# lim0606/pytorch-ardae-vae

Measured on AMD Instinct MI355X. Metric: AR-DAE-VAE train-steps/sec (batch 512, nz_cdae 256) on dbMNIST, higher is better.
Workload: dtype f32; 1 GPU; BASELINE config #2: MNISTIPVAE mlp z=32 h=256 + cDAE mlp-grad h=256 L=3, global batch 512, nz_cdae 256 (131072 rows), dynamic binarisation on device, 1 cDAE + 1 VAE update per step; global_batch=512, nz_cdae=256, per_gpu_batch=512, parallelism=dp1

## Files before the change

pytorch-ardae-vae_amd/csrc/wgrad_x9.hip:

```cpp
#include <stdlib.h>

#include <type_traits>

#include "profile.h"
#include "wgrad.h"
#include "wgrad_wide_tiles.h"

namespace ardae {
namespace {

typedef __bf16 bf16x8 __attribute__((ext_vector_type(8)));
typedef float f32x8 __attribute__((ext_vector_type(8)));

constexpr int XT = 256;
constexpr int XRC = 16;
constexpr int X_PLANE_BYTES = 2 * XT * 16;
constexpr int X_OP_BYTES = 3 * X_PLANE_BYTES;
constexpr int X_BUF_BYTES = 2 * X_OP_BYTES;

__device__ __forceinline__ void xload1(float& dst, unsigned voff, const float* sbase) {
  asm volatile("s_nop 4\n\tglobal_load_dword %0, %1, %2" : "+v"(dst) : "v"(voff), "s"(sbase) : "memory");
}
__device__ __forceinline__ void xload4(f32x4& dst, unsigned voff, const float* sbase) {
  asm volatile("s_nop 4\n\tglobal_load_dwordx4 %0, %1, %2" : "+v"(dst) : "v"(voff), "s"(sbase) : "memory");
}
template <int N>
__device__ __forceinline__ void xwait() { asm volatile("s_waitcnt vmcnt(%0)" : : "n"(N) : "memory"); }
__device__ __forceinline__ void take_landed(const float& loaded, unsigned& top, float& copy) {
  asm volatile("v_and_b32 %0, 0xffff0000, %2\n\tv_mov_b32 %1, %2" : "=&v"(top), "=&v"(copy) : "v"(loaded));
}
__device__ __forceinline__ void take_landed(const f32x4& loaded, f32x4& copy) {
  asm volatile("v_mov_b32 %0, %4\n\tv_mov_b32 %1, %5\n\tv_mov_b32 %2, %6\n\tv_mov_b32 %3, %7"
               : "=&v"(copy[0]), "=&v"(copy[1]), "=&v"(copy[2]), "=&v"(copy[3])
               : "v"(loaded[0]), "v"(loaded[1]), "v"(loaded[2]), "v"(loaded[3]));
}

struct Cut3 { unsigned h, m, l; };
__device__ __forceinline__ Cut3 cut3(float x) {
  Cut3 c;
  c.h = __float_as_uint(x) & 0xffff0000u;
  const float r1 = x - __uint_as_float(c.h);
  c.m = __float_as_uint(r1) & 0xffff0000u;
  c.l = __float_as_uint(r1 - __uint_as_float(c.m));
  return c;
}
__device__ __forceinline__ unsigned pack_hi(unsigned even, unsigned odd) { return __builtin_amdgcn_perm(odd, even, 0x07060302u); }
typedef unsigned u32x4 __attribute__((ext_vector_type(4)));

template <int N, class F>
__device__ __forceinline__ void static_for(F&& f) {
  if constexpr (N > 0) {
    static_for<N - 1>(f);
    f(std::integral_constant<int, N - 1>{});
  }
}
constexpr int X9_PA[9] = {2, 1, 2, 0, 2, 1, 0, 1, 0}, X9_PB[9] = {2, 2, 1, 2, 0, 1, 1, 0, 0};

struct X9Chunk {
  const float* g; const float* x; const float* rs;
  int ldg, ldx;
  float fb, fr;
};

__global__ __launch_bounds__(256, 1) void wgrad_x9_kernel(const WwBatchDev batch) {
  extern __shared__ __attribute__((aligned(16))) unsigned char lds[];
  const int tid = threadIdx.x, lane = tid & 63;
  const int wave = __builtin_amdgcn_readfirstlane(tid >> 6);
  const int l31 = lane & 31, hh = lane >> 5;
  const int wo = wave >> 1, wi = wave & 1;
  const int ti = (int)blockIdx.x / batch.splits, split = (int)blockIdx.x - ti * batch.splits;
  const WwTile T = batch.t[ti];

  const int cpp = T.M / XRC;
  const int ctot = cpp * T.npairs;
  const int cps = (ctot + batch.splits - 1) / batch.splits;
  const int c_begin = split * cps;
  const int c_end = c_begin + cps < ctot ? c_begin + cps : ctot;

  auto chunk_at = [&](int ch) {
    X9Chunk c;
    const int cc = ch < c_end ? ch : c_end - 1;
    const int pr = cc >= cpp ? 1 : 0;
    const int m0 = (cc - pr * cpp) * XRC;
    c.ldg = pr ? T.ldG[1] : T.ldG[0];
    c.ldx = pr ? T.ldX[1] : T.ldX[0];
    c.g = (pr ? T.G[1] : T.G[0]) + (size_t)m0 * c.ldg + T.o0;
    c.x = (pr ? T.X[1] : T.X[0]) + (size_t)m0 * c.ldx + T.i0;
    const bool vec = T.want_vec && pr == T.bias_pair && ch < c_end;
    c.fb = vec ? 1.f : 0.f;
    c.fr = (vec && T.rowscale) ? 1.f : 0.f;
    c.rs = T.rowscale ? T.rowscale + m0 : c.g;
    return c;
  };
  auto issue_loads = [&](const X9Chunk& c, float (&g)[XRC], float (&x)[XRC], f32x4 (&rs)[4]) {
    const float* pg = c.g;
    const float* px = c.x;
#pragma unroll
    for (int j = 0; j < XRC; ++j) {
      xload1(g[j], (unsigned)tid * 4u, pg); pg += c.ldg;
      if ((j & 3) == 3) xload4(rs[j >> 2], 0u, c.rs + (j & ~3));
    }
#pragma unroll
    for (int j = 0; j < XRC; ++j) { xload1(x[j], (unsigned)tid * 4u, px); px += c.ldx; }
  };
  float bsum = 0.f, rsum = 0.f;
  auto write_group = [&](const u32x4& h, const u32x4& m, const u32x4& l, int op, int kg, unsigned char* buf) {
    unsigned char* p = buf + op * X_OP_BYTES + (kg * XT + tid) * 16;
    *reinterpret_cast<u32x4*>(p) = h;
    *reinterpret_cast<u32x4*>(p + X_PLANE_BYTES) = m;
    *reinterpret_cast<u32x4*>(p + 2 * X_PLANE_BYTES) = l;
  };
  auto stage_group = [&](const float (&v)[XRC], int op, int kg, unsigned char* buf) {
    u32x4 h, m, l;
#pragma unroll
    for (int q = 0; q < 4; ++q) {
      const Cut3 e = cut3(v[8 * kg + 2 * q]), o = cut3(v[8 * kg + 2 * q + 1]);
      h[q] = pack_hi(e.h, o.h); m[q] = pack_hi(e.m, o.m); l[q] = pack_hi(e.l, o.l);
    }
    write_group(h, m, l, op, kg, buf);
  };

  f32x16 acc[4][4];
#pragma unroll
  for (int a = 0; a < 4; ++a)
#pragma unroll
    for (int b = 0; b < 4; ++b)
#pragma unroll
      for (int r = 0; r < 16; ++r) acc[a][b][r] = 0.f;

  if (c_begin < c_end) {
    float gc[XRC], xc[XRC];
    f32x4 rsc[4];
#pragma unroll
    for (int j = 0; j < XRC; ++j) gc[j] = xc[j] = 0.f;
#pragma unroll
    for (int q = 0; q < 4; ++q) rsc[q] = f32x4{0.f, 0.f, 0.f, 0.f};
    {
      const X9Chunk c0 = chunk_at(c_begin);
      issue_loads(c0, gc, xc, rsc);
      asm volatile("s_waitcnt vmcnt(0)" ::: "memory");
#pragma unroll
      for (int j = 0; j < XRC; ++j) asm volatile("" : "+v"(gc[j]), "+v"(xc[j]));
#pragma unroll
      for (int q = 0; q < 4; ++q) asm volatile("" : "+v"(rsc[q]));
      {
        float s0 = 0.f, r0 = 0.f;
#pragma unroll
        for (int j = 0; j < XRC; ++j) { s0 += gc[j]; r0 += gc[j] * rsc[j >> 2][j & 3]; }
        bsum += s0 * c0.fb; rsum += r0 * c0.fr;
      }
      stage_group(gc, 0, 0, lds); stage_group(gc, 0, 1, lds); stage_group(xc, 1, 0, lds); stage_group(xc, 1, 1, lds);
      issue_loads(chunk_at(c_begin + 1), gc, xc, rsc);
      __syncthreads();
    }
    int buf = 0;
    bf16x8 Af[3][4], Bf[3][4];
    auto read_plane = [&](auto pp, const unsigned char* from) {
      constexpr int p = decltype(pp)::value;
      static_for<4>([&](auto aa) {
        constexpr int a = decltype(aa)::value;
        Af[p][a] = *reinterpret_cast<const bf16x8*>(from + p * X_PLANE_BYTES + (hh * XT + wo * 128 + a * 32 + l31) * 16);
      });
      static_for<4>([&](auto bb) {
        constexpr int b = decltype(bb)::value;
        Bf[p][b] = *reinterpret_cast<const bf16x8*>(from + X_OP_BYTES + p * X_PLANE_BYTES + (hh * XT + wi * 128 + b * 32 + l31) * 16);
      });
    };
    using I0 = std::integral_constant<int, 0>;
    using I1 = std::integral_constant<int, 1>;
    using I2 = std::integral_constant<int, 2>;
    read_plane(I2{}, lds);
    read_plane(I1{}, lds);
    X9Chunk c1 = chunk_at(c_begin + 1);
#pragma unroll 1
    for (int ch = c_begin; ch < c_end; ++ch) {
      unsigned char* cur = lds + buf * X_BUF_BYTES;
      unsigned char* oth = lds + (buf ^ 1) * X_BUF_BYTES;
      const X9Chunk c2 = chunk_at(ch + 2);
      const float* pgn = c2.g;
      const float* pxn = c2.x;
      u32x4 sh, sm, sl;
      Cut3 ce{0u, 0u, 0u}, co{0u, 0u, 0u};
      float r1 = 0.f, vv = 0.f, cs = 0.f, cr = 0.f;
      f32x4 rsv = {0.f, 0.f, 0.f, 0.f};
      static_for<144>([&](auto nn) {
        constexpr int n = decltype(nn)::value, s = n >> 4, idx = n & 15, a = idx >> 2, b = idx & 3;
        acc[a][b] = __builtin_amdgcn_mfma_f32_32x32x16_bf16(Af[X9_PA[s]][a], Bf[X9_PB[s]][b], acc[a][b], 0, 0, 0);
        __builtin_amdgcn_sched_barrier(0);
        if constexpr (n == 0) {
          read_plane(I0{}, cur);
          __builtin_amdgcn_sched_barrier(0);
        }
        if constexpr (n < 124) {
          constexpr int grp = n / 31, r = n % 31;
          if constexpr (r < 28) {
            constexpr int pr = r / 7, slot = r % 7, e = 8 * grp + 2 * pr + (slot >= 3 ? 1 : 0), op = e >> 4, j = e & 15;
            float& v = op ? xc[j] : gc[j];
            if constexpr (slot == 0 || slot == 3) {
              xwait<35>();
              Cut3& c = slot == 0 ? ce : co;
              take_landed(v, c.h, vv);
              r1 = vv - __uint_as_float(c.h);
              if constexpr (op == 0) cs += vv;
            } else if constexpr (slot == 1 || slot == 4) {
              Cut3& c = slot == 1 ? ce : co;
              c.m = __float_as_uint(r1) & 0xffff0000u;
              c.l = __float_as_uint(r1 - __uint_as_float(c.m));
              if constexpr (op == 0) {
                if constexpr ((j & 3) == 0) { xwait<31>(); take_landed(rsc[j >> 2], rsv); }
                cr += vv * rsv[j & 3];
              }
            } else if constexpr (slot == 2 || slot == 5) {
              if constexpr (op == 0) {
                xload1(v, (unsigned)tid * 4u, pgn); pgn += c2.ldg;
                if constexpr ((j & 3) == 3) xload4(rsc[j >> 2], 0u, c2.rs + (j & ~3));
              } else {
                xload1(v, (unsigned)tid * 4u, pxn); pxn += c2.ldx;
              }
            } else {
              sh[pr] = pack_hi(ce.h, co.h); sm[pr] = pack_hi(ce.m, co.m); sl[pr] = pack_hi(ce.l, co.l);
            }
          } else {
            constexpr int pl = r - 28;
            unsigned char* p = oth + (grp >> 1) * X_OP_BYTES + ((grp & 1) * XT + tid) * 16 + pl * X_PLANE_BYTES;
            *reinterpret_cast<u32x4*>(p) = pl == 0 ? sh : pl == 1 ? sm : sl;
          }
          __builtin_amdgcn_sched_barrier(0);
        }
        if constexpr (n == 124) {
          __syncthreads();
          __builtin_amdgcn_sched_barrier(0);
        }
        if constexpr (n == 125) {
          read_plane(I2{}, oth);
          __builtin_amdgcn_sched_barrier(0);
        }
        if constexpr (n == 128) {
          read_plane(I1{}, oth);
          __builtin_amdgcn_sched_barrier(0);
        }
      });
      bsum += cs * c1.fb; rsum += cr * c1.fr;
      buf ^= 1;
      c1 = c2;
    }
    asm volatile("s_waitcnt vmcnt(0)" ::: "memory");
  }

  float* __restrict__ part = T.partial + (size_t)split * T.O * T.I;
#pragma unroll
  for (int a = 0; a < 4; ++a) {
#pragma unroll
    for (int b = 0; b < 4; ++b) {
      const int i = T.i0 + wi * 128 + b * 32 + l31;
#pragma unroll
      for (int r = 0; r < 16; ++r) {
        const int o = T.o0 + wo * 128 + a * 32 + (r & 3) + 8 * (r >> 2) + 4 * hh;
        part[(size_t)o * T.I + i] = acc[a][b][r];
      }
    }
  }
  if (T.want_vec && T.i0 == 0) {
    T.partial_vec[((size_t)split * 2 + 0) * T.O + T.o0 + tid] = bsum;
    T.partial_vec[((size_t)split * 2 + 1) * T.O + T.o0 + tid] = rsum;
  }
}

}

bool wgrad_x9_eligible(const WgradProblem& p) {
  static const bool off = debug_knob("ARDAE_WGRAD_X9") && atoi(debug_knob("ARDAE_WGRAD_X9")) == 0;
  if (off || p.O % XT || p.I % XT || p.M % XRC || p.M < 64 * 32) return false;
  for (int k = 0; k < p.npairs; ++k)
    if ((int64_t)p.ldG[k] * XRC * 4 >= (int64_t)1 << 31 || (int64_t)p.ldX[k] * XRC * 4 >= (int64_t)1 << 31) return false;
  return true;
}

int launch_wgrad_x9(const WwBatchDev& b, hipStream_t st) {
  static const bool attr_set = [] {
    return hipFuncSetAttribute(reinterpret_cast<const void*>(wgrad_x9_kernel), hipFuncAttributeMaxDynamicSharedMemorySize, 2 * X_BUF_BYTES) == hipSuccess;
  }();
  ARDAE_CHECK_ARG(attr_set, "wgrad_x9: cannot reserve %d bytes of LDS", 2 * X_BUF_BYTES);
  hipLaunchKernelGGL(wgrad_x9_kernel, dim3(b.ntiles * b.splits), dim3(256), 2 * X_BUF_BYTES, st, b);
  return 0;
}

}
```

Measured before the change: 223.7 train-steps/sec.

## Add 8-wave variant of x9 weight-gradient kernel and make it default

Adds a 512-thread version of the 3-way bf16-split weight-gradient MFMA kernel. Each wave now owns a 128x64 output sub-tile instead of 128x128, and half the waves stage G while the other half stage X, so per-thread global loads and split/pack work are halved. Row scales are read through scalar constant-address loads. The goal is more latency hiding and higher MFMA issue rate per CU. The cost is extra LDS A-fragment reads per MFMA and a barrier shared by more waves. The old 4-wave kernel can still be selected with a debug knob.

```diff
diff --git a/pytorch-ardae-vae_amd/csrc/wgrad_x9.hip b/pytorch-ardae-vae_amd/csrc/wgrad_x9.hip
--- a/pytorch-ardae-vae_amd/csrc/wgrad_x9.hip
+++ b/pytorch-ardae-vae_amd/csrc/wgrad_x9.hip
@@ -1,3 +1,4 @@
+#include <stdint.h>
 #include <stdlib.h>
 
 #include <type_traits>
@@ -46,6 +47,7 @@
 }
 __device__ __forceinline__ unsigned pack_hi(unsigned even, unsigned odd) { return __builtin_amdgcn_perm(odd, even, 0x07060302u); }
 typedef unsigned u32x4 __attribute__((ext_vector_type(4)));
+typedef __attribute__((address_space(4))) const float ConstF;
 
 template <int N, class F>
 __device__ __forceinline__ void static_for(F&& f) {
@@ -61,6 +63,39 @@
   int ldg, ldx;
   float fb, fr;
 };
+
+__device__ __forceinline__ X9Chunk x9_chunk_at(const WwTile& T, int ch, int c_end, int cpp) {
+  X9Chunk c;
+  const int cc = ch < c_end ? ch : c_end - 1;
+  const int pr = cc >= cpp ? 1 : 0;
+  const int m0 = (cc - pr * cpp) * XRC;
+  c.ldg = pr ? T.ldG[1] : T.ldG[0];
+  c.ldx = pr ? T.ldX[1] : T.ldX[0];
+  c.g = (pr ? T.G[1] : T.G[0]) + (size_t)m0 * c.ldg + T.o0;
+  c.x = (pr ? T.X[1] : T.X[0]) + (size_t)m0 * c.ldx + T.i0;
+  const bool vec = T.want_vec && pr == T.bias_pair && ch < c_end;
+  c.fb = vec ? 1.f : 0.f;
+  c.fr = (vec && T.rowscale) ? 1.f : 0.f;
+  c.rs = T.rowscale ? T.rowscale + m0 : c.g;
+  return c;
+}
+
+template <int NB>
+__device__ __forceinline__ void x9_store_partial(const WwTile& T, int split, const f32x16 (&acc)[4][NB], int o_w, int i_w, int l31, int hh) {
+  float* __restrict__ part = T.partial + (size_t)split * T.O * T.I;
+#pragma unroll
+  for (int a = 0; a < 4; ++a) {
+#pragma unroll
+    for (int b = 0; b < NB; ++b) {
+      const int i = T.i0 + i_w + b * 32 + l31;
+#pragma unroll
+      for (int r = 0; r < 16; ++r) {
+        const int o = T.o0 + o_w + a * 32 + (r & 3) + 8 * (r >> 2) + 4 * hh;
+        part[(size_t)o * T.I + i] = acc[a][b][r];
+      }
+    }
+  }
+}
 
 __global__ __launch_bounds__(256, 1) void wgrad_x9_kernel(const WwBatchDev batch) {
   extern __shared__ __attribute__((aligned(16))) unsigned char lds[];
@@ -77,21 +112,7 @@
   const int c_begin = split * cps;
   const int c_end = c_begin + cps < ctot ? c_begin + cps : ctot;
 
-  auto chunk_at = [&](int ch) {
-    X9Chunk c;
-    const int cc = ch < c_end ? ch : c_end - 1;
-    const int pr = cc >= cpp ? 1 : 0;
-    const int m0 = (cc - pr * cpp) * XRC;
-    c.ldg = pr ? T.ldG[1] : T.ldG[0];
-    c.ldx = pr ? T.ldX[1] : T.ldX[0];
-    c.g = (pr ? T.G[1] : T.G[0]) + (size_t)m0 * c.ldg + T.o0;
-    c.x = (pr ? T.X[1] : T.X[0]) + (size_t)m0 * c.ldx + T.i0;
-    const bool vec = T.want_vec && pr == T.bias_pair && ch < c_end;
-    c.fb = vec ? 1.f : 0.f;
-    c.fr = (vec && T.rowscale) ? 1.f : 0.f;
-    c.rs = T.rowscale ? T.rowscale + m0 : c.g;
-    return c;
-  };
+  auto chunk_at = [&](int ch) { return x9_chunk_at(T, ch, c_end, cpp); };
   auto issue_loads = [&](const X9Chunk& c, float (&g)[XRC], float (&x)[XRC], f32x4 (&rs)[4]) {
     const float* pg = c.g;
     const float* px = c.x;
@@ -247,22 +268,182 @@
     asm volatile("s_waitcnt vmcnt(0)" ::: "memory");
   }
 
-  float* __restrict__ part = T.partial + (size_t)split * T.O * T.I;
-#pragma unroll
-  for (int a = 0; a < 4; ++a) {
-#pragma unroll
-    for (int b = 0; b < 4; ++b) {
-      const int i = T.i0 + wi * 128 + b * 32 + l31;
-#pragma unroll
-      for (int r = 0; r < 16; ++r) {
-        const int o = T.o0 + wo * 128 + a * 32 + (r & 3) + 8 * (r >> 2) + 4 * hh;
-        part[(size_t)o * T.I + i] = acc[a][b][r];
-      }
-    }
-  }
+  x9_store_partial<4>(T, split, acc, wo * 128, wi * 128, l31, hh);
   if (T.want_vec && T.i0 == 0) {
     T.partial_vec[((size_t)split * 2 + 0) * T.O + T.o0 + tid] = bsum;
     T.partial_vec[((size_t)split * 2 + 1) * T.O + T.o0 + tid] = rsum;
+  }
+}
+
+__global__ __launch_bounds__(512, 1) void wgrad_x9_kernel_w8(const WwBatchDev batch) {
+  extern __shared__ __attribute__((aligned(16))) unsigned char lds[];
+  const int tid = threadIdx.x, lane = tid & 63, col = tid & 255;
+  const int wave = __builtin_amdgcn_readfirstlane(tid >> 6);
+  const int l31 = lane & 31, hh = lane >> 5;
+  const int op = wave >> 2;
+  const int wo = (wave >> 1) & 1, wi = 2 * (wave & 1) + op;
+  unsigned voff = (unsigned)col * 4u, rdA = (unsigned)(hh * XT + wo * 128 + l31) * 16u;
+  asm volatile("" : "+v"(voff), "+v"(rdA));
+  const int a2b = X_OP_BYTES + (wi * 64 - wo * 128) * 16, wr0 = op * X_OP_BYTES;
+  const int ti = (int)blockIdx.x / batch.splits, split = (int)blockIdx.x - ti * batch.splits;
+  const WwTile T = batch.t[ti];
+
+  const int cpp = T.M / XRC;
+  const int ctot = cpp * T.npairs;
+  const int cps = (ctot + batch.splits - 1) / batch.splits;
+  const int c_begin = split * cps;
+  const int c_end = c_begin + cps < ctot ? c_begin + cps : ctot;
+
+  auto chunk_at = [&](int ch) { return x9_chunk_at(T, ch, c_end, cpp); };
+  auto issue_loads = [&](const X9Chunk& c, float (&v)[XRC]) {
+    const float* p = op ? c.x : c.g;
+    const int ld = op ? c.ldx : c.ldg;
+#pragma unroll
+    for (int j = 0; j < XRC; ++j) { xload1(v[j], voff, p); p += ld; }
+  };
+  auto load_sigma = [&](const X9Chunk& c, float (&sg)[XRC]) {
+    const ConstF* rs = (const ConstF*)(uintptr_t)c.rs;
+    static_for<XRC>([&](auto jj) { sg[decltype(jj)::value] = rs[decltype(jj)::value]; });
+  };
+  float bsum = 0.f, rsum = 0.f;
+  auto stage_group = [&](const float (&v)[XRC], int kg, unsigned char* buf) {
+    u32x4 h, m, l;
+#pragma unroll
+    for (int q = 0; q < 4; ++q) {
+      const Cut3 e = cut3(v[8 * kg + 2 * q]), o = cut3(v[8 * kg + 2 * q + 1]);
+      h[q] = pack_hi(e.h, o.h); m[q] = pack_hi(e.m, o.m); l[q] = pack_hi(e.l, o.l);
+    }
+    unsigned char* p = buf + (voff * 4u + (unsigned)(wr0 + kg * XT * 16));
+    *reinterpret_cast<u32x4*>(p) = h;
+    *reinterpret_cast<u32x4*>(p + X_PLANE_BYTES) = m;
+    *reinterpret_cast<u32x4*>(p + 2 * X_PLANE_BYTES) = l;
+  };
+
+  f32x16 acc[4][2];
+#pragma unroll
+  for (int a = 0; a < 4; ++a)
+#pragma unroll
+    for (int b = 0; b < 2; ++b)
+#pragma unroll
+      for (int r = 0; r < 16; ++r) acc[a][b][r] = 0.f;
+
+  if (c_begin < c_end) {
+    float vc[XRC], sg[XRC];
+#pragma unroll
+    for (int j = 0; j < XRC; ++j) vc[j] = 0.f;
+    {
+      const X9Chunk c0 = chunk_at(c_begin);
+      issue_loads(c0, vc);
+      load_sigma(c0, sg);
+      asm volatile("s_waitcnt vmcnt(0)" ::: "memory");
+#pragma unroll
+      for (int j = 0; j < XRC; ++j) asm volatile("" : "+v"(vc[j]));
+      {
+        float s0 = 0.f, r0 = 0.f;
+#pragma unroll
+        for (int j = 0; j < XRC; ++j) { s0 += vc[j]; r0 += vc[j] * sg[j]; }
+        bsum += s0 * c0.fb; rsum += r0 * c0.fr;
+      }
+      stage_group(vc, 0, lds); stage_group(vc, 1, lds);
+      const X9Chunk cn = chunk_at(c_begin + 1);
+      issue_loads(cn, vc);
+      load_sigma(cn, sg);
+      __syncthreads();
+    }
+    int buf = 0;
+    bf16x8 Af[3][4], Bf[3][2];
+    auto read_plane = [&](auto pp, const unsigned char* from) {
+      constexpr int p = decltype(pp)::value;
+      static_for<4>([&](auto aa) {
+        constexpr int a = decltype(aa)::value;
+        Af[p][a] = *reinterpret_cast<const bf16x8*>(from + (rdA + (unsigned)(p * X_PLANE_BYTES + a * 512)));
+      });
+      static_for<2>([&](auto bb) {
+        constexpr int b = decltype(bb)::value;
+        Bf[p][b] = *reinterpret_cast<const bf16x8*>(from + a2b + (rdA + (unsigned)(p * X_PLANE_BYTES + b * 512)));
+      });
+    };
+    using I0 = std::integral_constant<int, 0>;
+    using I1 = std::integral_constant<int, 1>;
+    using I2 = std::integral_constant<int, 2>;
+    read_plane(I2{}, lds);
+    read_plane(I1{}, lds);
+    X9Chunk c1 = chunk_at(c_begin + 1);
+#pragma unroll 1
+    for (int ch = c_begin; ch < c_end; ++ch) {
+      unsigned char* cur = lds + buf * X_BUF_BYTES;
+      unsigned char* oth = lds + (buf ^ 1) * X_BUF_BYTES;
+      const X9Chunk c2 = chunk_at(ch + 2);
+      const float* pn = op ? c2.x : c2.g;
+      const int ldn = op ? c2.ldx : c2.ldg;
+      u32x4 sh, sm, sl;
+      Cut3 ce{0u, 0u, 0u}, co{0u, 0u, 0u};
+      float r1 = 0.f, cs = 0.f, cr = 0.f;
+      static_for<72>([&](auto nn) {
+        constexpr int n = decltype(nn)::value, s = n >> 3, idx = n & 7, a = idx >> 1, b = idx & 1;
+        acc[a][b] = __builtin_amdgcn_mfma_f32_32x32x16_bf16(Af[X9_PA[s]][a], Bf[X9_PB[s]][b], acc[a][b], 0, 0, 0);
+        __builtin_amdgcn_sched_barrier(0);
+        if constexpr (n == 0) {
+          read_plane(I0{}, cur);
+          __builtin_amdgcn_sched_barrier(0);
+        }
+        if constexpr (n < 62) {
+          constexpr int kg = n / 31, r = n % 31;
+          if constexpr (r < 28) {
+            constexpr int pr = r / 7, slot = r % 7, j = 8 * kg + 2 * pr + (slot >= 3 ? 1 : 0);
+            float& v = vc[j];
+            if constexpr (slot == 0 || slot == 3) {
+              xwait<15>();
+              Cut3& c = slot == 0 ? ce : co;
+              asm volatile("v_and_b32 %0, 0xffff0000, %3\n\tv_sub_f32 %1, %3, %0\n\tv_add_f32 %2, %2, %3" : "=&v"(c.h), "=&v"(r1), "+v"(cs) : "v"(v));
+            } else if constexpr (slot == 1 || slot == 4) {
+              Cut3& c = slot == 1 ? ce : co;
+              c.m = __float_as_uint(r1) & 0xffff0000u;
+              c.l = __float_as_uint(r1 - __uint_as_float(c.m));
+              float t;
+              asm volatile("v_mul_f32 %1, %3, %2\n\tv_add_f32 %0, %0, %1" : "+v"(cr), "=&v"(t) : "v"(v), "s"(sg[j]));
+            } else if constexpr (slot == 2 || slot == 5) {
+              xload1(v, voff, pn); pn += ldn;
+            } else {
+              sh[pr] = pack_hi(ce.h, co.h); sm[pr] = pack_hi(ce.m, co.m); sl[pr] = pack_hi(ce.l, co.l);
+            }
+          } else {
+            constexpr int pl = r - 28;
+            unsigned char* p = oth + wr0 + (voff * 4u + (unsigned)(kg * XT * 16 + pl * X_PLANE_BYTES));
+            *reinterpret_cast<u32x4*>(p) = pl == 0 ? sh : pl == 1 ? sm : sl;
+          }
+          __builtin_amdgcn_sched_barrier(0);
+        }
+        if constexpr (n == 62) {
+          __syncthreads();
+          __builtin_amdgcn_sched_barrier(0);
+        }
+        if constexpr (n == 63) {
+          read_plane(I2{}, oth);
+          __builtin_amdgcn_sched_barrier(0);
+        }
+        if constexpr (n == 64) {
+          read_plane(I1{}, oth);
+          __builtin_amdgcn_sched_barrier(0);
+        }
+        if constexpr (n == 66) {
+          load_sigma(c2, sg);
+          __builtin_amdgcn_sched_barrier(0);
+        }
+      });
+      bsum += cs * c1.fb; rsum += cr * c1.fr;
+      buf ^= 1;
+      c1 = c2;
+    }
+    asm volatile("s_waitcnt vmcnt(0)" ::: "memory");
+  }
+
+  asm volatile("" : "+v"(voff));
+  const int colS = (int)(voff >> 2), laneS = colS & 63;
+  x9_store_partial<2>(T, split, acc, wo * 128, wi * 64, laneS & 31, laneS >> 5);
+  if (T.want_vec && T.i0 == 0 && op == 0) {
+    T.partial_vec[((size_t)split * 2 + 0) * T.O + T.o0 + colS] = bsum;
+    T.partial_vec[((size_t)split * 2 + 1) * T.O + T.o0 + colS] = rsum;
   }
 }
 
@@ -278,10 +459,15 @@
 
 int launch_wgrad_x9(const WwBatchDev& b, hipStream_t st) {
   static const bool attr_set = [] {
-    return hipFuncSetAttribute(reinterpret_cast<const void*>(wgrad_x9_kernel), hipFuncAttributeMaxDynamicSharedMemorySize, 2 * X_BUF_BYTES) == hipSuccess;
+    return hipFuncSetAttribute(reinterpret_cast<const void*>(wgrad_x9_kernel), hipFuncAttributeMaxDynamicSharedMemorySize, 2 * X_BUF_BYTES) == hipSuccess &&
+           hipFuncSetAttribute(reinterpret_cast<const void*>(wgrad_x9_kernel_w8), hipFuncAttributeMaxDynamicSharedMemorySize, 2 * X_BUF_BYTES) == hipSuccess;
   }();
   ARDAE_CHECK_ARG(attr_set, "wgrad_x9: cannot reserve %d bytes of LDS", 2 * X_BUF_BYTES);
-  hipLaunchKernelGGL(wgrad_x9_kernel, dim3(b.ntiles * b.splits), dim3(256), 2 * X_BUF_BYTES, st, b);
+  const char* waves = debug_knob("ARDAE_X9_WAVES");
+  if (waves && atoi(waves) == 4)
+    hipLaunchKernelGGL(wgrad_x9_kernel, dim3(b.ntiles * b.splits), dim3(256), 2 * X_BUF_BYTES, st, b);
+  else
+    hipLaunchKernelGGL(wgrad_x9_kernel_w8, dim3(b.ntiles * b.splits), dim3(512), 2 * X_BUF_BYTES, st, b);
   return 0;
 }
 
```

Measured after the change: 225.2 train-steps/sec (median of 6 runs). No clear change (+0.7%).
